# roclark/torchsr

Measured on AMD Instinct MI355X. Metric: 96x96 HR crops/sec (SRGAN GAN train step), higher is better.
Workload: dtype f32; 1 GPU; SRGAN full GAN step (Generator + Discriminator + VGG19 perceptual loss), 96x96 HR crops, batch 16 per GPU, fp32; per_gpu_batch=16, global_batch=16, crop=96, parallelism=dp1, hip_graph=True, vgg19_weights=seeded-random, plan_cus=256

## Files before the change

include/srx.h:

```cpp
#ifndef SRX_H
#define SRX_H

#include <stddef.h>
#include <stdint.h>

#ifdef __cplusplus
extern "C" {
#endif

#define SRX_VERSION 100

enum {
  SRX_OK = 0,
  SRX_E_BADARG = 1,
  SRX_E_UNSUPPORTED = 2,
  SRX_E_HIP = 3,
  SRX_E_WORKSPACE = 4
};

enum { SRX_ACT_NONE = 0, SRX_ACT_RELU = 1, SRX_ACT_LRELU = 2, SRX_ACT_PRELU = 3 };

int srx_version(void);
int srx_last_error(char* buf, size_t n);
int srx_build_info(char* buf, size_t n);
// ... 33 lines not shown
  int32_t up;
  int32_t precision;
} srx_conv2d_t;

size_t srx_conv2d_packed_fwd_floats(const srx_conv2d_t* d);
size_t srx_conv2d_packed_bwd_floats(const srx_conv2d_t* d);
size_t srx_conv2d_fwd_ws_floats(const srx_conv2d_t* d);
size_t srx_conv2d_bwd_data_ws_floats(const srx_conv2d_t* d);
size_t srx_conv2d_bwd_weight_ws_floats(const srx_conv2d_t* d);
int srx_conv2d_stat_rows(const srx_conv2d_t* d);

int srx_conv2d_plan(const srx_conv2d_t* d, int which, int* out);

int srx_conv2d_force_plan(int bm, int bn, int split, int ks);
int srx_conv2d_force_s2(int mode, int bm, int bn);
int srx_wgrad_force(int lin, int nsplit);
int srx_wgrad_force_kernels(int dma, int rows, int reduce);
int srx_thin_force_rows(int rows);
int srx_linear_force(int form, int splits);

int srx_thin_plan(const srx_conv2d_t* d, int which, int* out);

int srx_linear_plan(int B, int K, int J, int which, int* out);

int srx_wgrad_plan(const srx_conv2d_t* d, int nprob, int per_out, int* out);

int srx_conv2d_pack(const srx_conv2d_t* d, const float* w_oihw, float* wpk_fwd, float* wpk_bwd, void* stream);

size_t srx_pack_table_bytes(int n_layers);
int srx_pack_table_build(const srx_conv2d_t* descs, int n, const float* const* w_oihw, float* const* wpk_fwd,
// ... 279 lines not shown
```

torchsr_amd/_lib.py:

```python
import ctypes as C
import os
import subprocess
import sys

_HERE = os.path.dirname(os.path.abspath(__file__))
CSRC = os.path.join(_HERE, 'csrc')
LIB_PATH = os.environ.get('SRX_LIB') or os.path.join(CSRC, 'libsrx_hip.so')
SOURCES = ['api.cpp', 'gconv.hip', 'wgrad.hip', 'convpack.hip', 'c64.hip', 'thin9.hip', 'rdb.hip', 'thin.hip', 'rowtile.hip', 'augment.hip', 'degrade.hip', 'norm.hip', 'eltwise.hip', 'linear.hip', 'loss.hip', 'head.hip', 'wino.hip', 'optim.hip', 'dihedral.hip', 'resample.hip', 'usm.hip', 'pool.hip', 'colorfix.hip', 'compact.hip', 'specnorm.hip']
HEADERS = ['srx_common.h', 'conv_host.h', os.path.join('..', '..', 'include', 'srx.h')]

ACT_NONE, ACT_RELU, ACT_LRELU, ACT_PRELU = 0, 1, 2, 3


class Conv2dDesc(C.Structure):
    _fields_ = [
        ('N', C.c_int32), ('H', C.c_int32), ('W', C.c_int32),
        ('Cin', C.c_int32), ('Cin_s', C.c_int32), ('Cout', C.c_int32), ('Cout_s', C.c_int32),
        ('KH', C.c_int32), ('KW', C.c_int32), ('stride', C.c_int32), ('pad', C.c_int32),
        ('shuffle', C.c_int32), ('act', C.c_int32), ('slope', C.c_float), ('up', C.c_int32),
        ('precision', C.c_int32),
    ]


class DgradEpilogue(C.Structure):
# ... 118 lines not shown
    'srx_color_fix_wavelet_level': (_I, [_P, _P, _P, _P, _L, _I, _I, _I, _P]),
    'srx_plane_moments_blocks': (_I, [_I, _I]),
    'srx_plane_moments': (_I, [_P, _L, _I, _I, _P, _Z, _P, _P]),
    'srx_color_fix_adain_apply': (_I, [_P, _P, _L, _I, _I, _P, _P, _P]),
    'srx_conv2d_packed_fwd_floats': (_Z, [_D]),
    'srx_conv2d_packed_bwd_floats': (_Z, [_D]),
    'srx_conv2d_fwd_ws_floats': (_Z, [_D]),
    'srx_conv2d_bwd_data_ws_floats': (_Z, [_D]),
    'srx_conv2d_bwd_weight_ws_floats': (_Z, [_D]),
    'srx_conv2d_stat_rows': (_I, [_D]),
    'srx_conv2d_plan': (_I, [_D, _I, C.POINTER(C.c_int)]),
    'srx_conv2d_force_plan': (_I, [_I, _I, _I, _I]),
    'srx_thin_plan': (_I, [_D, _I, C.POINTER(C.c_int)]),
    'srx_thin_force_rows': (_I, [_I]),
    'srx_conv2d_force_s2': (_I, [_I, _I, _I]),
    'srx_wgrad_force': (_I, [_I, _I]),
    'srx_wgrad_force_kernels': (_I, [_I, _I, _I]),
    'srx_wgrad_plan': (_I, [_D, _I, _I, C.POINTER(C.c_int)]),
    'srx_linear_force': (_I, [_I, _I]),
    'srx_linear_plan': (_I, [_I, _I, _I, _I, C.POINTER(C.c_int)]),
    'srx_pack_table_bytes': (_Z, [_I]),
    'srx_pack_table_build': (_I, [_P, _I, _P, _P, _P, _P, C.POINTER(C.c_int), C.POINTER(C.c_longlong)]),
    'srx_pack_table_add_wino': (_I, [_P, C.POINTER(C.c_int), C.POINTER(C.c_longlong), _D, _P, _P, _I]),
    'srx_pack_table_run': (_I, [_P, _I, C.c_longlong, _P]),
    'srx_conv2d_pack': (_I, [_D, _P, _P, _P, _P]),
    'srx_conv2d_fwd': (_I, [_D, _P, _P, _P, _P, _P, _P, _Z, _P]),
    'srx_conv3x3_c64_bf16_packed_bytes': (_Z, [_I]),
    'srx_conv3x3_c64_bf16_pack': (_I, [_P, _P, _P, _I, _I, _P, _P]),
    'srx_conv3x3_c64_bf16_fwd': (_I, [_I, _I, _I, _I, _I, _P, _P, _F, _P, _P, _I, _P]),
    'srx_conv3x3_c64_bf16_plan': (_I, [_I, _I, _I, _I, C.POINTER(C.c_int)]),
# ... 202 lines not shown
```

torchsr_amd/csrc/api.cpp:

```cpp
#include "srx_common.h"
#include <cstdarg>
#include <cstdio>
#include <atomic>
#include <cstdlib>
#include <cstring>
#include <mutex>
#include <vector>

static thread_local char g_err[512] = "";

void srx_set_error(const char* fmt, ...) {
  va_list ap;
  va_start(ap, fmt);
  vsnprintf(g_err, sizeof(g_err), fmt, ap);
  va_end(ap);
}

extern "C" int srx_version(void) { return SRX_VERSION; }

#ifndef SRX_SOURCES_SHA256
#define SRX_SOURCES_SHA256 "unknown"
#endif
static const char g_build_info[] = "srx-build-sources-sha256:" SRX_SOURCES_SHA256;
extern "C" int srx_build_info(char* buf, size_t n) {
// ... 3 lines not shown
  return SRX_OK;
}

static SrxDevSwitches read_switches() {
  SrxDevSwitches s{};
  auto flag = [](const char* n) { const char* e = getenv(n); return e != nullptr && e[0] != 0 && !(e[0] == '0' && e[1] == 0); };
  auto num = [](const char* n) { const char* e = getenv(n); return e ? atoi(e) : 0; };
  s.no_rt36 = flag("SRX_NO_RT36");
  s.no_wgrad_rows = flag("SRX_NO_WGRAD_ROWS");
  s.no_bn_bwd_fuse = flag("SRX_NO_BN_BWD_FUSE");
  s.no_bn_fwd_fuse = flag("SRX_NO_BN_FWD_FUSE");
  s.no_first3 = flag("SRX_NO_FIRST3");
  s.no_c64 = flag("SRX_NO_C64");
  s.no_wgrad_dma = flag("SRX_NO_WGRAD_DMA");
  s.no_wgrad_lin = flag("SRX_NO_WGRAD_LIN");
  s.wgrad_nsplit = num("SRX_WGRAD_NSPLIT");
  s.wgrad_rows_nsplit = num("SRX_WGRAD_ROWS_NSPLIT");
  s.first3_wgs_per_cu = num("SRX_FIRST3_WGS_PER_CU");
  s.thin_fwd_rows = num("SRX_THIN_FWD_ROWS");
  s.reserved_cus = num("SRX_RESERVED_CUS");
  s.c64_ablate = num("SRX_C64_ABLATE");
  s.rdb_ablate = num("SRX_RDB_ABLATE");
  s.no_wino = flag("SRX_NO_WINO");
  s.old_wgrad_reduce = flag("SRX_OLD_WGRAD_REDUCE");
  s.wino_no_tail = flag("SRX_WINO_NO_TAIL");
  s.wino_zsplit = num("SRX_WINO_ZSPLIT");
  s.wino_bn = num("SRX_WINO_BN");
  s.s2_mode = num("SRX_S2_MODE");
  if (s.rdb_ablate != 0 || s.c64_ablate != 0) {
    const char* ok = getenv("SRX_ALLOW_GARBAGE_RESULTS");
// ... 142 lines not shown
```

torchsr_amd/csrc/conv_host.h:

```cpp
#pragma once
#include "srx_common.h"
#include <atomic>

constexpr int BK = 32;

struct Geo {
  int Ho, Wo, Ck, K, Kp, Cnp, cps;
};

struct BwdClass {
  int ph, pw, nth, ntw, dminh, dminw, Hm, Wm, K, Kp;
  size_t woff;
};

int check_desc(const srx_conv2d_t* d);
bool small_enough(const srx_conv2d_t* d);
int pad_rows(int c);
Geo fwd_geo(const srx_conv2d_t* d);
int bwd_ck(const srx_conv2d_t* d);
int bwd_classes(const srx_conv2d_t* d, BwdClass* cls, size_t& total_floats);
srx_conv2d_t upsampled_desc(const srx_conv2d_t* d);
size_t upsampled_floats(const srx_conv2d_t* d);

struct ConvForce {
  std::atomic<int> plan[4];
  std::atomic<int> s2[3];
  std::atomic<int> wg[2];
  std::atomic<int> wg_rows;
  std::atomic<int> wk[3];
};
ConvForce& conv_force();
```

torchsr_amd/csrc/gconv.hip:

```cpp
#include "conv_host.h"
#include <cstdio>
#include <cstdlib>
#include <algorithm>
#include <mutex>
#include <type_traits>
#include <utility>
#include <vector>

namespace {

struct GArgs {
  const float* in; const float* w; const float* bias; float* out; float* part;
  int N, Hi, Wi, Ci;
  int Hm, Wm, M, HmWm;
  float inv_HmWm, inv_Wm;
  int in_stride, nth, ntw, dh0, dw0, Ck, K, Kp;
  int Cn, Cs;
  int Ho, Wo, Co;
  int out_stride, oh_off, ow_off;
  int out_shuffle, in_shuffle;
  int up;
  int act; float slope;
  int linear_out;
  int mtiles;
// ... 3 lines not shown
  unsigned w_bytes;
  int big;
  unsigned in_margin;
  const float* add;
  float oscale;
  int add_ld, add_hi;
  float ascale;
  const float* mask;
  float mask_slope;
  int mask_lo, mask_hi;
  int out16, mask16;
};

constexpr int INVALID = -20000;

template <int BM, int BN, int WM, int WN, int KS, int XR, int PR, int UP = 0, int BIG = 0>
__device__ __forceinline__ void gconv_body(const GArgs& a, const int bid) {
  static_assert(XR == 0 || (XR == 16 && KS == 1), "extra rows: 16, without the in-workgroup K split");
  static_assert(PR == 0 || XR == 0, "the 16-row extension is fp32 only");
  constexpr bool H16 = PR == 1 || PR == 3;
  constexpr int BKL = H16 ? BK / 2 : BK;
  constexpr int NS = H16 ? 2 : 4;
  constexpr int BMT = BM + XR;
  constexpr int TM = WM / 32, TN = WN / 32;
  constexpr int WAVES_N = BN / WN;
  constexpr int WAVES_M = BM / WM;
  constexpr int GT = WAVES_M * WAVES_N * 64;
  constexpr int NT = GT * KS;
  static_assert(NT == 256 || NT == 512, "4 or 8 waves per workgroup");
  constexpr int RPP = GT / 8;
  constexpr int RA = (BMT + RPP - 1) / RPP, RB = BN / RPP;
  static_assert(RA >= 1 && RB >= 1, "tile too small for the thread count");
// ... 44 lines not shown
  size_t tbase = 0;
  if constexpr (BIG) {
    int n, mh, mw;
    split_row(min(m0, a.M - 1), n, mh, mw);
    const size_t c0 = centre(n, mh * a.in_stride, mw * a.in_stride);
    tbase = c0 > a.in_margin ? c0 - a.in_margin : 0;
    const unsigned tb_in_lo = (unsigned)srx_uniform((int)(unsigned)(tbase & 0xffffffffu));
    const unsigned tb_in_hi = (unsigned)srx_uniform((int)(unsigned)(tbase >> 32));
    tbase = ((size_t)tb_in_hi << 32) | tb_in_lo;
  }
  const size_t in_left = a.in_bytes - tbase;
  const __amdgpu_buffer_rsrc_t rin = BIG ? srx_rsrc(reinterpret_cast<const char*>(a.in) + tbase, in_left > 0xfffffff0ull ? 0xfffffff0u : (unsigned)in_left)
                                         : srx_rsrc(a.in, (unsigned)a.in_bytes);
  const __amdgpu_buffer_rsrc_t rw = srx_rsrc(a.w, a.w_bytes);

  for (int e = kc_beg * 8 + (int)threadIdx.x; e < kc_end * 8; e += NT) {
    const int k = 4 * e;
    int2 ent;
    if (k < a.K) {
      const int tap = k / a.Ck, c = k - tap * a.Ck;
      const int th = tap / a.ntw, tw = tap - th * a.ntw;
      const int dh = a.dh0 + th, dw = a.dw0 + tw;
      int koff;
      if (UP) {
        koff = c;
      } else if (a.in_shuffle) {
        const int ij = c / a.in_shuffle, cc = c - ij * a.in_shuffle;
        koff = ((2 * dh + (ij >> 1)) * (2 * a.Wi) + 2 * dw + (ij & 1)) * a.Ci + cc;
      } else {
        koff = (dh * a.Wi + dw) * a.Ci + c;
      }
      ent.x = (int)((unsigned)(dh & 0xffff) | ((unsigned)dw << 16));
      ent.y = koff * 4;
    } else {
      ent.x = (INVALID & 0xffff);
      ent.y = 0;
    }
    ktab[e - kc_beg * 8] = ent;
  }

  int rih[RA], riw[RA];
  unsigned rbase[RA];
#pragma unroll
  for (int p = 0; p < RA; ++p) {
    const int m = m0 + r0 + RPP * p;
    if (m < a.M && r0 + RPP * p < BMT) {
      int n, mh, mw;
      split_row(m, n, mh, mw);
      const int ih0 = mh * a.in_stride, iw0 = mw * a.in_stride;
      rih[p] = ih0;
      riw[p] = iw0;
      if constexpr (BIG) {
        rbase[p] = (unsigned)(centre(n, ih0, iw0) - tbase);
      } else {
        rbase[p] = 4u * (unsigned)(UP ? n * (a.Hi >> 1) * (a.Wi >> 1) * a.Ci
                                   : a.in_shuffle ? ((n * 2 * a.Hi + 2 * ih0) * (2 * a.Wi) + 2 * iw0) * a.Ci
                                                  : ((n * a.Hi + ih0) * a.Wi + iw0) * a.Ci);
      }
    } else {
      rih[p] = INVALID; riw[p] = 0; rbase[p] = 0;
    }
  }
  unsigned wvoff[RB];
#pragma unroll
  for (int p = 0; p < RB; ++p) wvoff[p] = 4u * ((unsigned)(n0 + r0 + RPP * p) * (unsigned)a.Kp + q * 4);
  __syncthreads();

  f32x16 acc[TM][TN];
#pragma unroll
  for (int i = 0; i < TM; ++i)
#pragma unroll
    for (int j = 0; j < TN; ++j)
#pragma unroll
      for (int r = 0; r < 16; ++r) acc[i][j][r] = 0.f;

  f32x4 ra0[RA], rb0[RB], ra1[RA], rb1[RB], ra2[RA], rb2[RB];
  auto gload = [&](int kc, f32x4 (&ra)[RA], f32x4 (&rb)[RB]) {
    const bool live = kc < kc_end;
    const int2 kt = ktab[(live ? kc - kc_beg : 0) * 8 + q];
    const int dh = (int)(short)(kt.x & 0xffff), dw = kt.x >> 16;
    if (UP) {
#pragma unroll
      for (int p = 0; p < RA; ++p) {
        const int ih = rih[p] + dh, iw = riw[p] + dw;
        const bool ok = live && ((unsigned)ih < (unsigned)a.Hi) && ((unsigned)iw < (unsigned)a.Wi);
        const unsigned pix = 4u * (unsigned)(((ih >> 1) * (a.Wi >> 1) + (iw >> 1)) * a.Ci);
        ra[p] = srx_bload(rin, ok ? rbase[p] + pix + (unsigned)kt.y : 0xffffffffu, 0);
      }
    } else {
#pragma unroll
      for (int p = 0; p < RA; ++p) {
        const int ih = rih[p] + dh, iw = riw[p] + dw;
        const bool ok = live && ((unsigned)ih < (unsigned)a.Hi) && ((unsigned)iw < (unsigned)a.Wi);
// ... 368 lines not shown
    }
    __syncthreads();
    if (lead && tid < BN) {
      float s = 0.f, s2 = 0.f;
#pragma unroll
      for (int w = 0; w < RED_ROWS; ++w) { s += red[(w * BN + tid) * 2]; s2 += red[(w * BN + tid) * 2 + 1]; }
      const int col = n0 + tid;
      if (col < a.Cn) {
        a.part[((size_t)mt * a.Cn + col) * 2 + 0] = s;
        a.part[((size_t)mt * a.Cn + col) * 2 + 1] = s2;
      }
    }
  }
}

template <int BM, int BN, int WM, int WN, int KS, int XR, int PR, int BIG = 0>
__global__ __launch_bounds__((BM / WM) * (BN / WN) * 64 * KS) void gconv_kernel(const GArgs a) {
  if (a.up) gconv_body<BM, BN, WM, WN, KS, XR, PR, 1, BIG>(a, blockIdx.x);
  else gconv_body<BM, BN, WM, WN, KS, XR, PR, 0, BIG>(a, blockIdx.x);
}

struct GMulti {
  int n;
  int first[5];
  GArgs g[4];
};
template <int BM, int BN, int WM, int WN, int XR, int PR = 0, int KS = 1>
__global__ __launch_bounds__((BM / WM) * (BN / WN) * 64 * KS) void gconv_multi_kernel(const GMulti m) {
  int ci = 0;
  while (ci + 1 < m.n && (int)blockIdx.x >= m.first[ci + 1]) ++ci;
  const GArgs a = m.g[ci];
  gconv_body<BM, BN, WM, WN, KS, XR, PR>(a, blockIdx.x - m.first[ci]);
}

struct S2Class {
  int nth, ntw, dh0, dw0;
  int chunks, pstart;
  int oh_off, ow_off;
  unsigned wbase, kpb;
};
struct GFused {
  GArgs g;
  int nclass, cpt, ptotal;
  S2Class c[4];
};

template <int BM, int BN, int WM, int WN, int XR, int PR>
// ... 479 lines not shown
srx_conv2d_t upsampled_desc(const srx_conv2d_t* d) {
  srx_conv2d_t h = *d;
  h.up = 0; h.H = 2 * d->H; h.W = 2 * d->W;
  return h;
}
size_t upsampled_floats(const srx_conv2d_t* d) { return (size_t)d->N * 2 * d->H * 2 * d->W * d->Cin_s; }

ConvForce& conv_force() {
  static ConvForce* f = [] {
    ConvForce* s = new ConvForce;
    const SrxDevSwitches& e = srx_dev();
    for (int i = 0; i < 4; ++i) s->plan[i].store(e.force_plan ? e.plan[i] : 0);
    s->s2[0].store((e.s2_mode & 1) ? 1 : 0); s->s2[1].store(0); s->s2[2].store(0);
    s->wg[0].store(e.no_wgrad_lin ? 0 : -1); s->wg[1].store(e.wgrad_nsplit > 0 && e.wgrad_nsplit <= 64 ? e.wgrad_nsplit : 0);
    s->wg_rows.store(e.wgrad_rows_nsplit > 0 && e.wgrad_rows_nsplit <= 64 ? e.wgrad_rows_nsplit : 0);
    s->wk[0].store(e.no_wgrad_dma ? 0 : -1); s->wk[1].store(e.no_wgrad_rows ? 0 : -1); s->wk[2].store(e.old_wgrad_reduce ? 0 : -1);
    return s;
  }();
  return *f;
}

namespace {

struct Plan { int BM, BN, mtiles, ntiles, tiles, full, tail, split, kc_per_split, ks; float cost; bool refused; };

enum Family { F_GCONV, F_BIG, F_MULTI, F_S2F, NFAM };
constexpr unsigned char K1 = 1, K2 = 2, K4 = 4, K12 = K1 | K2;
struct Tile {
  int BM, BN, WM, WN, XR;
  float eff;
  unsigned char ks[NFAM][4];
};
constexpr Tile kTiles[] = {
    {144, 128, 64, 32, 16, 0.91f, {{K1}, {}, {K1}, {K1}}},
    {144, 64, 32, 32, 16, 0.82f, {{K1}, {}, {K1}, {K1}}},
    {128, 128, 64, 32, 0, 0.95f, {{K1, K1, K1, K1}, {K1, K1, 0, K1}, {K1, K1}, {K1, K1}}},
    {128, 64, 32, 32, 0, 0.85f, {{K1, K1, K1, K1}, {K1, K1, 0, K1}, {K1, K1}, {K1, K1}}},
    {64, 64, 32, 32, 0, 0.60f, {{K12, K12, K12, K12}, {}, {K12, K12}, {K1, K1}}},
    {128, 32, 32, 32, 0, 0.50f, {{K1, K1, 0, K1}, {K1, K1, 0, K1}, {K1, K1}, {}}},
    {64, 32, 32, 32, 0, 0.50f, {{K2, K4, 0, K4}}},
    {256, 128, 64, 64, 0, 1.08f, {{0, K1, K1, K1}}},
};
constexpr int NTILES = sizeof(kTiles) / sizeof(kTiles[0]);

const Tile* find_tile(int bm, int bn) {
  const Tile* t = std::find_if(kTiles, kTiles + NTILES, [&](const Tile& x) { return x.BM == bm && x.BN == bn; });
  return t != kTiles + NTILES ? t : nullptr;
}
bool has_tile(Family f, int bm, int bn, int ks, int pr) {
  const Tile* t = find_tile(bm, bn);
  return t && (t->ks[f][pr] & (ks ? ks : K1 | K2 | K4)) != 0;
}
bool tile_sides_known(Family f, int bm, int bn) {
  bool rows = false, cols = false;
  for (const Tile& t : kTiles)
    if (t.ks[f][0] | t.ks[f][1] | t.ks[f][2] | t.ks[f][3]) { rows |= t.BM == bm; cols |= t.BN == bn; }
  return rows && cols;
}
int tile_ks(const Tile& t, Family f, int pr, bool two) {
  const int have = t.ks[f][pr];
  return have == K12 ? (two ? 2 : 1) : have ? have : 1;
}
bool columns_fit(int Cnp, int bn) { return Cnp == 32 ? bn == 32 : (bn != 32 && Cnp % bn == 0); }

float tile_us(int bm, int bn, int chunks, float eff, bool bf16) {
  return 2.0f * bm * bn * (float)chunks * BK / (4 * 64 * 2.1e3f) / eff / (bf16 ? 3.0f : 1.0f);
}
// ... 57 lines not shown
      return p;
    }
    p.BM = bm; p.BN = bn; p.mtiles = (int)srx_cdiv(M, bm); p.ntiles = Cnp / bn; p.tiles = p.mtiles * p.ntiles;
    if (sp > 1 && can_split) { p.full = 0; p.tail = p.tiles; p.kc_per_split = (int)srx_cdiv(kchunks, sp); p.split = (int)srx_cdiv(kchunks, p.kc_per_split); }
    else { p.full = p.tiles; p.tail = 0; p.split = 1; p.kc_per_split = kchunks; }
    p.ks = tile_ks(*find_tile(bm, bn), F_GCONV, pr, ks == 2);
    return p;
  }
  const Tile* t = find_tile(best.BM, best.BN);
  best.ks = t ? tile_ks(*t, fam, pr, best.full + best.tail * best.split <= P && best.kc_per_split >= 4) : 1;
  return best;
}

size_t plan_ws_floats(const Plan& p) { return p.split > 1 ? (size_t)p.tail * p.split * p.BM * p.BN : 0; }

template <int BM, int BN, int WM, int WN, int KS, int XR, int PR = 0, int BIG = 0>
int launch_gconv(const GArgs& a, const Plan& p, hipStream_t st) {
  const int ktab_chunks = p.full > 0 || p.split == 1 ? a.kchunks : p.kc_per_split;
  const size_t lds = gconv_lds_bytes(BM + XR, BN, KS, PR, ktab_chunks);
  if (lds > 160 * 1024) SRX_FAIL(SRX_E_UNSUPPORTED, "conv2d: K range needs %zu bytes of LDS", lds);
  static std::once_flag once;
  std::call_once(once, [] {
    (void)hipFuncSetAttribute(reinterpret_cast<const void*>(&gconv_kernel<BM, BN, WM, WN, KS, XR, PR, BIG>),
                              hipFuncAttributeMaxDynamicSharedMemorySize, 160 * 1024);
  });
  dim3 grid(p.full + p.tail * p.split);
  char nm[112];
  if (srx_prof_on())
    snprintf(nm, sizeof(nm), "gconv_kernel<%d, %d, %d, %d, %d, %d, %d%s> MxNxK=%dx%dx%d", BM, BN, WM, WN, KS, XR, PR, BIG ? ", big" : "",
             a.M, a.Cn, PR == 2 ? 2 * a.K : a.K);
  SRX_LAUNCH_PROF(nm, 2.0 * a.M * a.Cn * (PR == 2 ? 2 * a.K : a.K), (gconv_kernel<BM, BN, WM, WN, KS, XR, PR, BIG>), grid,
                  dim3((BM / WM) * (BN / WN) * 64 * KS), lds, st, a);
  SRX_CHECK_LAUNCH("gconv_kernel");
  if (p.split > 1) {
    hipLaunchKernelGGL((tail_fixup_kernel<BM + XR, BN>), dim3(p.tail * (BN / 16)), dim3(256), 0, st, a);
    SRX_CHECK_LAUNCH("tail_fixup_kernel");
  }
  return SRX_OK;
}

template <int BM, int BN, int WM, int WN, int XR, int PR = 0, int KS = 1>
int launch_gconv_multi(const GMulti& m, size_t lds, hipStream_t st) {
  static std::once_flag once;
  std::call_once(once, [] {
    (void)hipFuncSetAttribute(reinterpret_cast<const void*>(&gconv_multi_kernel<BM, BN, WM, WN, XR, PR, KS>),
                              hipFuncAttributeMaxDynamicSharedMemorySize, 160 * 1024);
  });
  char nm[64];
  double fl = 0.0;
  if (srx_prof_on()) {
    snprintf(nm, sizeof(nm), "gconv_multi_kernel<%d, %d, %d, %d, %d, %d, %d>", BM, BN, WM, WN, XR, PR, KS);
    for (int i = 0; i < m.n; ++i) fl += 2.0 * m.g[i].M * m.g[i].Cn * m.g[i].K;
  }
  SRX_LAUNCH_PROF(nm, fl, (gconv_multi_kernel<BM, BN, WM, WN, XR, PR, KS>), dim3(m.first[m.n]), dim3((BM / WM) * (BN / WN) * 64 * KS),
                  lds, st, m);
  SRX_CHECK_LAUNCH("gconv_multi_kernel");
  return SRX_OK;
}

template <int BM, int BN, int WM, int WN, int XR, int PR>
int launch_gconv_s2f(const GFused& f, dim3 grid, size_t lds, double fl, hipStream_t st) {
  static std::once_flag once;
  std::call_once(once, [] {
    (void)hipFuncSetAttribute(reinterpret_cast<const void*>(&gconv_s2f_kernel<BM, BN, WM, WN, XR, PR>),
                              hipFuncAttributeMaxDynamicSharedMemorySize, 160 * 1024);
  });
  char nm[64];
  if (srx_prof_on()) snprintf(nm, sizeof(nm), "gconv_s2f_kernel<%d, %d, %d, %d, %d, %d>", BM, BN, WM, WN, XR, PR);
  SRX_LAUNCH_PROF(nm, fl, (gconv_s2f_kernel<BM, BN, WM, WN, XR, PR>), grid, dim3((BM / WM) * (BN / WN) * 64), lds, st, f);
  SRX_CHECK_LAUNCH("gconv_s2f_kernel");
  return SRX_OK;
}

struct TileKey { int bm, bn, ks, pr; };

template <int F, int I, int PR, int KS, class... A>
bool launch_if(const TileKey& k, int& rc, const A&... args) {
  constexpr Tile t = kTiles[I];
  if constexpr ((t.ks[F][PR] & KS) != 0) {
    if (k.bm != t.BM || k.bn != t.BN || k.ks != KS || k.pr != PR) return false;
    if constexpr (F == F_MULTI) rc = launch_gconv_multi<t.BM - t.XR, t.BN, t.WM, t.WN, t.XR, PR, KS>(args...);
    else if constexpr (F == F_S2F) rc = launch_gconv_s2f<t.BM - t.XR, t.BN, t.WM, t.WN, t.XR, PR>(args...);
    else rc = launch_gconv<t.BM - t.XR, t.BN, t.WM, t.WN, KS, t.XR, PR, F == F_BIG>(args...);
    return true;
  }
  return false;
}
using Listable = std::make_integer_sequence<int, NTILES * 12>;
template <int F, int... J, class... A>
bool launch_tile(std::integer_sequence<int, J...>, const TileKey& k, int& rc, const A&... args) {
  return (launch_if<F, J / 12, J / 3 % 4, 1 << J % 3>(k, rc, args...) || ...);
}

// ... 30 lines not shown
        const float t = tile_us(bm, bn, kch, 1.0f, bf16);
        const float cost = ks == 2 ? 6.5f + 0.5f * t / 0.8f : 1.0f + t / tile.eff;
        const int tiles = (int)srx_cdiv(m.g[c].M, bm) * (int)srx_cdiv(m.g[c].Cn, bn);
        for (int t = 0; t < tiles; ++t) {
          std::pop_heap(heap.begin(), heap.end(), later);
          heap.back() += cost;
          if (heap.back() > makespan) makespan = heap.back();
          std::push_heap(heap.begin(), heap.end(), later);
        }
      }
    if (makespan < best) { best = makespan; BM = bm; BN = bn; KS = ks; }
  }
  return best;
}

int run_gconv_multi(GMulti& m, int BM, int BN, int KS, hipStream_t st, int precision = 0) {
  std::stable_sort(m.g, m.g + m.n, [](const GArgs& x, const GArgs& y) { return x.Kp > y.Kp; });
  int maxk = 0;
  m.first[0] = 0;
  for (int i = 0; i < m.n; ++i) {
    GArgs& a = m.g[i];
    a.kchunks = a.Kp / BK;
    a.mtiles = (int)srx_cdiv(a.M, BM);
    a.kc_per_split = a.kchunks;
    a.tail_split = 1;
    a.ws = nullptr;
    const int tiles = a.mtiles * (int)srx_cdiv(a.Cn, BN);
    a.full_tiles = tiles;
    m.first[i + 1] = m.first[i] + tiles;
    if (a.kchunks > maxk) maxk = a.kchunks;
  }
  const int pr = precision ? 1 : 0;
  const size_t lds = gconv_lds_bytes(BM, BN, KS, pr, maxk);
  if (lds > 160 * 1024) SRX_FAIL(SRX_E_UNSUPPORTED, "conv2d: K range needs %zu bytes of LDS", lds);
  int rc = SRX_OK;
  if (launch_tile<F_MULTI>(Listable{}, {BM, BN, KS, pr}, rc, m, lds, st)) return rc;
  SRX_FAIL(SRX_E_UNSUPPORTED, "conv2d_bwd_data: no%s gconv_multi_kernel for tile %d x %d", pr ? " bf16" : "", BM, BN);
}

bool s2f_eligible(const srx_conv2d_t* d, const BwdClass* cls, int nc) {
  if (nc < 2 || nc > 4 || d->shuffle || d->up || d->precision > 1) return false;
  if (bwd_ck(d) % BK != 0 || pad_rows(d->Cin) % 64 != 0) return false;
  for (int i = 0; i < nc; ++i)
    if (cls[i].K == 0 || cls[i].Hm != cls[0].Hm || cls[i].Wm != cls[0].Wm || cls[i].Hm <= 0 || cls[i].Wm <= 0) return false;
  return true;
}

float s2f_tile(const srx_conv2d_t* d, const BwdClass* cls, int nc, int& BM, int& BN) {
  const int P = srx_plan_cus();
  const bool bf16 = d->precision != 0;
  const int Cnp = pad_rows(d->Cin);
// ... 29 lines not shown
    S2Class& k = f.c[i];
    k.nth = cls[i].nth; k.ntw = cls[i].ntw; k.dh0 = cls[i].dminh; k.dw0 = cls[i].dminw;
    k.chunks = cls[i].K / BK; k.pstart = pos;
    k.oh_off = cls[i].ph; k.ow_off = cls[i].pw;
    k.wbase = (unsigned)(cls[i].woff * sizeof(float)); k.kpb = (unsigned)(cls[i].Kp * sizeof(float));
    pos += (int)srx_roundup(k.chunks, 3);
    fl += 2.0 * shared.M * shared.Cn * cls[i].K;
  }
  f.ptotal = pos;
  const int Cnp = pad_rows(d->Cin);
  const int pr = d->precision != 0 ? 1 : 0;
  const size_t lds = s2f_lds_bytes(BM, BN, pr, pos);
  if (lds > 160 * 1024) SRX_FAIL(SRX_E_UNSUPPORTED, "conv2d_bwd_data: K range needs %zu bytes of LDS", lds);
  const dim3 grid((unsigned)(f.g.mtiles * (Cnp / BN)));
  int rc = SRX_OK;
  if (launch_tile<F_S2F>(Listable{}, {BM, BN, 1, pr}, rc, f, grid, lds, fl, st)) return rc;
  SRX_FAIL(SRX_E_UNSUPPORTED, "conv2d_bwd_data: internal: no fused-class instantiation for tile %d x %d", BM, BN);
}

int strided_dgrad_plan(const srx_conv2d_t* d, const BwdClass* cls, int nc, const GMulti& m, int& BM, int& BN, int& KS, bool& fused) {
  ConvForce& f = conv_force();
  const int mode = f.s2[0].load(std::memory_order_relaxed);
  const bool bf16 = d->precision != 0;
  const int Cnp = pad_rows(d->Cin);
  const bool eligible = m.n == nc && s2f_eligible(d, cls, nc);
  fused = false;
  if (mode == 2) {
    if (!eligible)
      SRX_FAIL(SRX_E_UNSUPPORTED, "conv2d_bwd_data: forced gconv_s2f_kernel refused: the layer needs 2..4 non-empty stride-parity "
                                  "classes on one grid (extents multiples of the stride), Cout and Cin in whole chunks, no shuffle / upsample");
    int bm = f.s2[1].load(std::memory_order_relaxed), bn = f.s2[2].load(std::memory_order_relaxed);
// ... 23 lines not shown
int run_gconv(GArgs& a, const Plan& p, float* ws, size_t ws_floats, hipStream_t st, int precision = 0) {
  if (p.refused) return SRX_E_UNSUPPORTED;
  a.kchunks = a.Kp / BK;
  const size_t need = plan_ws_floats(p);
  if (need && (!ws || need > ws_floats))
    SRX_FAIL(SRX_E_WORKSPACE, "conv2d: split-K workspace %zu < %zu floats", ws_floats, need);
  if (p.split > 1 && !a.linear_out) SRX_FAIL(SRX_E_UNSUPPORTED, "conv2d: internal: split plan on a strided output");
  a.mtiles = p.mtiles;
  a.kc_per_split = p.kc_per_split;
  a.full_tiles = p.full;
  a.tail_split = p.split;
  a.ws = ws;
  int rc = SRX_OK;
  if (a.big) {
    if (p.split > 1) SRX_FAIL(SRX_E_UNSUPPORTED, "conv2d: internal: split plan on a call above 2^24 pixels");
    if (launch_tile<F_BIG>(Listable{}, {p.BM, p.BN, p.ks, precision == 3 ? 3 : precision ? 1 : 0}, rc, a, p, st)) return rc;
    SRX_FAIL(SRX_E_UNSUPPORTED, "conv2d: no whole-frame kernel for tile %dx%d", p.BM, p.BN);
  }
  if (launch_tile<F_GCONV>(Listable{}, {p.BM, p.BN, p.ks, precision}, rc, a, p, st)) return rc;
  static const char* const arith[4] = {"fp32", "bf16", "bf16-storage", "fp16"};
  SRX_FAIL(SRX_E_UNSUPPORTED, "conv2d: no %s kernel for tile %dx%d", arith[precision & 3], p.BM, p.BN);
}

void set_mgrid(GArgs& a, int N, int Hm, int Wm) {
  a.N = N; a.Hm = Hm; a.Wm = Wm; a.HmWm = Hm * Wm; a.M = N * Hm * Wm;
  a.inv_HmWm = 1.0f / (float)a.HmWm;
  a.inv_Wm = 1.0f / (float)Wm;
}

bool is_big(const srx_conv2d_t* d) { return !small_enough(d); }

Plan fwd_plan(const srx_conv2d_t* d, const Geo& g) {
  return make_plan(d->N * g.Ho * g.Wo, g.Cnp, g.Kp / BK, !d->shuffle, d->precision != 0, is_big(d));
}
// ... 98 lines not shown
              (tile_sides_known(F_GCONV, bm, bn) && split >= 1 && split <= 16 && (ks == 1 || ks == 2)),
              "conv2d_force_plan: (0, 0, 0, 0) or BM 64 / 128 / 144 / 256, BN 32 / 64 / 128, split 1..16, KS 1 / 2");
  ConvForce& f = conv_force();
  f.plan[1].store(0);
  f.plan[0].store(bm); f.plan[2].store(split); f.plan[3].store(ks); f.plan[1].store(bn);
  return SRX_OK;
}

extern "C" int srx_conv2d_force_s2(int mode, int bm, int bn) {
  SRX_REQUIRE(((mode == 0 || mode == 1) && bm == 0 && bn == 0) ||
              (mode == 2 && ((bm == 0 && bn == 0) || tile_sides_known(F_S2F, bm, bn))),
              "conv2d_force_s2: (0, 0, 0), (1, 0, 0) or (2, BM 64 / 128 / 144, BN 64 / 128) -- (2, 0, 0): the model's fused tile");
  ConvForce& f = conv_force();
  f.s2[0].store(0);
  f.s2[1].store(bm); f.s2[2].store(bn); f.s2[0].store(mode);
  return SRX_OK;
}

extern "C" int srx_wgrad_force(int lin, int nsplit) {
  SRX_REQUIRE(lin >= -1 && lin <= 1 && nsplit >= 0 && nsplit <= 64, "wgrad_force: LIN -1 / 0 / 1, 0..64 row splits");
  ConvForce& f = conv_force();
  f.wg[0].store(lin); f.wg[1].store(nsplit); f.wg_rows.store(nsplit);
  return SRX_OK;
}

extern "C" int srx_wgrad_force_kernels(int dma, int rows, int reduce) {
  SRX_REQUIRE(dma >= -1 && dma <= 1 && rows >= -1 && rows <= 1 && reduce >= -1 && reduce <= 1,
              "wgrad_force_kernels: DMA staging, image-row kernel, row-wise reduction: each -1 / 0 / 1");
  ConvForce& f = conv_force();
  f.wk[0].store(dma); f.wk[1].store(rows); f.wk[2].store(reduce);
// ... 367 lines not shown
```

torchsr_amd/csrc/srx_common.h:

```cpp
#pragma once
#include <hip/hip_runtime.h>
#include <hip/hip_ext.h>
#include <stdint.h>
#include <stddef.h>
#include "../../include/srx.h"

typedef float f32x4 __attribute__((ext_vector_type(4)));
typedef float f32x16 __attribute__((ext_vector_type(16)));

void srx_set_error(const char* fmt, ...);

#define SRX_FAIL(code, ...)      \
  do {                           \
    srx_set_error(__VA_ARGS__);  \
    return (code);               \
  } while (0)

#define SRX_REQUIRE(cond, ...) \
  do {                         \
    if (!(cond)) SRX_FAIL(SRX_E_BADARG, __VA_ARGS__); \
  } while (0)

#define SRX_CHECK_LAUNCH(name)                                                        \
  do {                                                                                \
    hipError_t e__ = hipGetLastError();                                               \
    if (e__ != hipSuccess) SRX_FAIL(SRX_E_HIP, "%s: %s", name, hipGetErrorString(e__)); \
  } while (0)

struct SrxDevSwitches {
  bool no_rt36, no_wgrad_rows, no_bn_bwd_fuse, no_bn_fwd_fuse, no_first3, no_c64, force_plan, no_wgrad_dma, no_wgrad_lin, no_wino, old_wgrad_reduce, wino_no_tail;
  int wgrad_nsplit, wgrad_rows_nsplit, first3_wgs_per_cu, thin_fwd_rows, reserved_cus, c64_ablate, rdb_ablate, wino_zsplit, wino_bn;
  int s2_mode;
  int plan[4];
};
const SrxDevSwitches& srx_dev();
extern "C" int srx_plan_cus(void);

bool srx_prof_on();
bool srx_prof_aux();
bool srx_prof_take(const char* name, double flops, hipEvent_t* e0, hipEvent_t* e1);
#define SRX_LAUNCH_PROF(name, flops, kernel, grid, block, lds, st, ...)                              \
  do {                                                                                               \
    hipEvent_t e0__ = nullptr, e1__ = nullptr;                                                       \
    if (srx_prof_on() && srx_prof_take(name, flops, &e0__, &e1__))                                   \
      hipExtLaunchKernelGGL(kernel, grid, block, (std::uint32_t)(lds), st, e0__, e1__, 0, __VA_ARGS__); \
// ... 91 lines not shown
```

Measured before the change: 2433 crops/s.

## Add tabled gather loader to gconv replacing LDS k-table with register tap walk

Adds a TAB variant of the implicit-GEMM conv body for plain fp32 non-upsampled convolutions. Instead of building a per-chunk (dh,dw) offset table in LDS and reading it on every load, each thread precomputes a per-row bitmask of in-image taps and walks tap/channel-chunk counters in scalar registers, using an out-of-range buffer offset to zero padding taps. The variant is enabled by default only for the 144-row tiles (single conv and multi-class dgrad) and can be disabled with an environment switch. It trades LDS traffic and address arithmetic for extra registers and is limited to at most 32 taps and Ck divisible by BK.

```diff
diff --git a/include/srx.h b/include/srx.h
--- a/include/srx.h
+++ b/include/srx.h
@@ -71,6 +71,8 @@
 
 int srx_conv2d_force_plan(int bm, int bn, int split, int ks);
 int srx_conv2d_force_s2(int mode, int bm, int bn);
+int srx_conv2d_force_gather(int tab);
+int srx_conv2d_gather_plan(const srx_conv2d_t* d, int which, int* out);
 int srx_wgrad_force(int lin, int nsplit);
 int srx_wgrad_force_kernels(int dma, int rows, int reduce);
 int srx_thin_force_rows(int rows);
diff --git a/torchsr_amd/_lib.py b/torchsr_amd/_lib.py
--- a/torchsr_amd/_lib.py
+++ b/torchsr_amd/_lib.py
@@ -156,6 +156,8 @@
     'srx_thin_plan': (_I, [_D, _I, C.POINTER(C.c_int)]),
     'srx_thin_force_rows': (_I, [_I]),
     'srx_conv2d_force_s2': (_I, [_I, _I, _I]),
+    'srx_conv2d_force_gather': (_I, [_I]),
+    'srx_conv2d_gather_plan': (_I, [_D, _I, C.POINTER(C.c_int)]),
     'srx_wgrad_force': (_I, [_I, _I]),
     'srx_wgrad_force_kernels': (_I, [_I, _I, _I]),
     'srx_wgrad_plan': (_I, [_D, _I, _I, C.POINTER(C.c_int)]),
diff --git a/torchsr_amd/csrc/api.cpp b/torchsr_amd/csrc/api.cpp
--- a/torchsr_amd/csrc/api.cpp
+++ b/torchsr_amd/csrc/api.cpp
@@ -41,6 +41,7 @@
   s.no_c64 = flag("SRX_NO_C64");
   s.no_wgrad_dma = flag("SRX_NO_WGRAD_DMA");
   s.no_wgrad_lin = flag("SRX_NO_WGRAD_LIN");
+  s.no_gather_tab = flag("SRX_NO_GATHER_TAB");
   s.wgrad_nsplit = num("SRX_WGRAD_NSPLIT");
   s.wgrad_rows_nsplit = num("SRX_WGRAD_ROWS_NSPLIT");
   s.first3_wgs_per_cu = num("SRX_FIRST3_WGS_PER_CU");
diff --git a/torchsr_amd/csrc/conv_host.h b/torchsr_amd/csrc/conv_host.h
--- a/torchsr_amd/csrc/conv_host.h
+++ b/torchsr_amd/csrc/conv_host.h
@@ -25,6 +25,7 @@
 struct ConvForce {
   std::atomic<int> plan[4];
   std::atomic<int> s2[3];
+  std::atomic<int> tab;
   std::atomic<int> wg[2];
   std::atomic<int> wg_rows;
   std::atomic<int> wk[3];
diff --git a/torchsr_amd/csrc/gconv.hip b/torchsr_amd/csrc/gconv.hip
--- a/torchsr_amd/csrc/gconv.hip
+++ b/torchsr_amd/csrc/gconv.hip
@@ -41,8 +41,9 @@
 
 constexpr int INVALID = -20000;
 
-template <int BM, int BN, int WM, int WN, int KS, int XR, int PR, int UP = 0, int BIG = 0>
+template <int BM, int BN, int WM, int WN, int KS, int XR, int PR, int UP = 0, int BIG = 0, int TAB = 0>
 __device__ __forceinline__ void gconv_body(const GArgs& a, const int bid) {
+  static_assert(TAB == 0 || (PR == 0 && UP == 0 && BIG == 0), "the tabled loader: plain fp32 gathers below 2^24 pixels");
   static_assert(XR == 0 || (XR == 16 && KS == 1), "extra rows: 16, without the in-workgroup K split");
   static_assert(PR == 0 || XR == 0, "the 16-row extension is fp32 only");
   constexpr bool H16 = PR == 1 || PR == 3;
@@ -117,7 +118,7 @@
                                          : srx_rsrc(a.in, (unsigned)a.in_bytes);
   const __amdgpu_buffer_rsrc_t rw = srx_rsrc(a.w, a.w_bytes);
 
-  for (int e = kc_beg * 8 + (int)threadIdx.x; e < kc_end * 8; e += NT) {
+  for (int e = kc_beg * 8 + (int)threadIdx.x; !TAB && e < kc_end * 8; e += NT) {
     const int k = 4 * e;
     int2 ent;
     if (k < a.K) {
@@ -144,6 +145,12 @@
 
   int rih[RA], riw[RA];
   unsigned rbase[RA];
+  int rout_of[RA];
+  unsigned rows1 = 0;
+  if constexpr (TAB) {
+    for (int th = 0; th < a.nth; ++th) rows1 |= 1u << (th * a.ntw);
+  }
+  auto below = [](int n) -> unsigned { return (unsigned)((1ull << n) - 1ull); };
 #pragma unroll
   for (int p = 0; p < RA; ++p) {
     const int m = m0 + r0 + RPP * p;
@@ -153,7 +160,15 @@
       const int ih0 = mh * a.in_stride, iw0 = mw * a.in_stride;
       rih[p] = ih0;
       riw[p] = iw0;
-      if constexpr (BIG) {
+      if constexpr (TAB) {
+        const int eh = ih0 + a.dh0, ew = iw0 + a.dw0;
+        const int hl = min(max(-eh, 0), a.nth), hh = max(min(a.Hi - eh, a.nth), hl);
+        const int wl = min(max(-ew, 0), a.ntw), wh = max(min(a.Wi - ew, a.ntw), wl);
+        const unsigned wbits = below(wh) & ~below(wl);
+        const unsigned in_img = (wbits * rows1) & below(hh * a.ntw) & ~below(hl * a.ntw);
+        rout_of[p] = (int)~in_img;
+        rbase[p] = 4u * (unsigned)(((n * a.Hi + ih0) * a.Wi + iw0) * a.Ci) + 16u * (unsigned)q;
+      } else if constexpr (BIG) {
         rbase[p] = (unsigned)(centre(n, ih0, iw0) - tbase);
       } else {
         rbase[p] = 4u * (unsigned)(UP ? n * (a.Hi >> 1) * (a.Wi >> 1) * a.Ci
@@ -162,7 +177,19 @@
       }
     } else {
       rih[p] = INVALID; riw[p] = 0; rbase[p] = 0;
-    }
+      if constexpr (TAB) rout_of[p] = -1;
+    }
+  }
+  const int cpt = TAB ? a.Ck / BK : 1;
+  int tb_t = 0, tb_th = 0, tb_tw = 0, tb_c = 0;
+  int tb_ones = -1;
+  if constexpr (TAB) asm("" : "+s"(tb_ones));
+  if constexpr (TAB) {
+    const int first = kc_beg + ks;
+    tb_t = srx_uniform(first / cpt);
+    tb_c = first - tb_t * cpt;
+    tb_th = srx_uniform(tb_t / a.ntw);
+    tb_tw = tb_t - tb_th * a.ntw;
   }
   unsigned wvoff[RB];
 #pragma unroll
@@ -180,6 +207,23 @@
   f32x4 ra0[RA], rb0[RB], ra1[RA], rb1[RB], ra2[RA], rb2[RB];
   auto gload = [&](int kc, f32x4 (&ra)[RA], f32x4 (&rb)[RB]) {
     const bool live = kc < kc_end;
+    if constexpr (TAB) {
+      const unsigned koff = 4u * (unsigned)(((a.dh0 + tb_th) * a.Wi + a.dw0 + tb_tw) * a.Ci + tb_c * BK);
+      const int dead = live ? 0 : tb_ones;
+#pragma unroll
+      for (int p = 0; p < RA; ++p)
+        ra[p] = srx_bload(rin, (rbase[p] + koff) | (unsigned)(__builtin_amdgcn_sbfe(rout_of[p], (unsigned)tb_t, 1u) | dead), 0);
+#pragma unroll
+      for (int p = 0; p < RB; ++p)
+        rb[p] = srx_bload(rw, live ? wvoff[p] : 0xffffffffu, (unsigned)srx_uniform(live ? kc * (BK * 4) : 0));
+#pragma unroll
+      for (int i = 0; i < KS; ++i)
+        if (++tb_c == cpt) {
+          tb_c = 0; ++tb_t;
+          if (++tb_tw == a.ntw) { tb_tw = 0; ++tb_th; }
+        }
+      return;
+    }
     const int2 kt = ktab[(live ? kc - kc_beg : 0) * 8 + q];
     const int dh = (int)(short)(kt.x & 0xffff), dw = kt.x >> 16;
     if (UP) {
@@ -578,8 +622,9 @@
   }
 }
 
-template <int BM, int BN, int WM, int WN, int KS, int XR, int PR, int BIG = 0>
+template <int BM, int BN, int WM, int WN, int KS, int XR, int PR, int BIG = 0, int TAB = 0>
 __global__ __launch_bounds__((BM / WM) * (BN / WN) * 64 * KS) void gconv_kernel(const GArgs a) {
+  if constexpr (TAB) { gconv_body<BM, BN, WM, WN, KS, XR, PR, 0, BIG, 1>(a, blockIdx.x); return; }
   if (a.up) gconv_body<BM, BN, WM, WN, KS, XR, PR, 1, BIG>(a, blockIdx.x);
   else gconv_body<BM, BN, WM, WN, KS, XR, PR, 0, BIG>(a, blockIdx.x);
 }
@@ -589,12 +634,12 @@
   int first[5];
   GArgs g[4];
 };
-template <int BM, int BN, int WM, int WN, int XR, int PR = 0, int KS = 1>
+template <int BM, int BN, int WM, int WN, int XR, int PR = 0, int KS = 1, int TAB = 0>
 __global__ __launch_bounds__((BM / WM) * (BN / WN) * 64 * KS) void gconv_multi_kernel(const GMulti m) {
   int ci = 0;
   while (ci + 1 < m.n && (int)blockIdx.x >= m.first[ci + 1]) ++ci;
   const GArgs a = m.g[ci];
-  gconv_body<BM, BN, WM, WN, KS, XR, PR>(a, blockIdx.x - m.first[ci]);
+  gconv_body<BM, BN, WM, WN, KS, XR, PR, 0, 0, TAB>(a, blockIdx.x - m.first[ci]);
 }
 
 struct S2Class {
@@ -1104,6 +1149,7 @@
     s->s2[0].store((e.s2_mode & 1) ? 1 : 0); s->s2[1].store(0); s->s2[2].store(0);
     s->wg[0].store(e.no_wgrad_lin ? 0 : -1); s->wg[1].store(e.wgrad_nsplit > 0 && e.wgrad_nsplit <= 64 ? e.wgrad_nsplit : 0);
     s->wg_rows.store(e.wgrad_rows_nsplit > 0 && e.wgrad_rows_nsplit <= 64 ? e.wgrad_rows_nsplit : 0);
+    s->tab.store(e.no_gather_tab ? 0 : -1);
     s->wk[0].store(e.no_wgrad_dma ? 0 : -1); s->wk[1].store(e.no_wgrad_rows ? 0 : -1); s->wk[2].store(e.old_wgrad_reduce ? 0 : -1);
     return s;
   }();
@@ -1120,16 +1166,17 @@
   int BM, BN, WM, WN, XR;
   float eff;
   unsigned char ks[NFAM][4];
+  unsigned char tab[2];
 };
 constexpr Tile kTiles[] = {
-    {144, 128, 64, 32, 16, 0.91f, {{K1}, {}, {K1}, {K1}}},
-    {144, 64, 32, 32, 16, 0.82f, {{K1}, {}, {K1}, {K1}}},
-    {128, 128, 64, 32, 0, 0.95f, {{K1, K1, K1, K1}, {K1, K1, 0, K1}, {K1, K1}, {K1, K1}}},
-    {128, 64, 32, 32, 0, 0.85f, {{K1, K1, K1, K1}, {K1, K1, 0, K1}, {K1, K1}, {K1, K1}}},
-    {64, 64, 32, 32, 0, 0.60f, {{K12, K12, K12, K12}, {}, {K12, K12}, {K1, K1}}},
-    {128, 32, 32, 32, 0, 0.50f, {{K1, K1, 0, K1}, {K1, K1, 0, K1}, {K1, K1}, {}}},
-    {64, 32, 32, 32, 0, 0.50f, {{K2, K4, 0, K4}}},
-    {256, 128, 64, 64, 0, 1.08f, {{0, K1, K1, K1}}},
+    {144, 128, 64, 32, 16, 0.91f, {{K1}, {}, {K1}, {K1}}, {K1, K1}},
+    {144, 64, 32, 32, 16, 0.82f, {{K1}, {}, {K1}, {K1}}, {K1, K1}},
+    {128, 128, 64, 32, 0, 0.95f, {{K1, K1, K1, K1}, {K1, K1, 0, K1}, {K1, K1}, {K1, K1}}, {}},
+    {128, 64, 32, 32, 0, 0.85f, {{K1, K1, K1, K1}, {K1, K1, 0, K1}, {K1, K1}, {K1, K1}}, {}},
+    {64, 64, 32, 32, 0, 0.60f, {{K12, K12, K12, K12}, {}, {K12, K12}, {K1, K1}}, {}},
+    {128, 32, 32, 32, 0, 0.50f, {{K1, K1, 0, K1}, {K1, K1, 0, K1}, {K1, K1}, {}}, {}},
+    {64, 32, 32, 32, 0, 0.50f, {{K2, K4, 0, K4}}, {}},
+    {256, 128, 64, 64, 0, 1.08f, {{0, K1, K1, K1}}, {}},
 };
 constexpr int NTILES = sizeof(kTiles) / sizeof(kTiles[0]);
 
@@ -1141,6 +1188,18 @@
   const Tile* t = find_tile(bm, bn);
   return t && (t->ks[f][pr] & (ks ? ks : K1 | K2 | K4)) != 0;
 }
+bool has_tab_tile(Family f, int bm, int bn, int ks) {
+  const Tile* t = find_tile(bm, bn);
+  return t && (f == F_GCONV || f == F_MULTI) && (t->tab[f == F_MULTI] & ks) != 0;
+}
+bool gather_tab_eligible(int precision, int in_shuffle, int up, int big, int Ck, int taps) {
+  return precision == 0 && !in_shuffle && !up && !big && Ck % BK == 0 && taps >= 1 && taps <= 32;
+}
+bool gather_tab_eligible(const GArgs& a, int precision) {
+  return gather_tab_eligible(precision, a.in_shuffle, a.up, a.big, a.Ck, a.nth * a.ntw) && a.K == a.Kp;
+}
+bool gather_tab_wanted() { return conv_force().tab.load(std::memory_order_relaxed) != 0; }
+
 bool tile_sides_known(Family f, int bm, int bn) {
   bool rows = false, cols = false;
   for (const Tile& t : kTiles)
@@ -1228,14 +1287,14 @@
 
 size_t plan_ws_floats(const Plan& p) { return p.split > 1 ? (size_t)p.tail * p.split * p.BM * p.BN : 0; }
 
-template <int BM, int BN, int WM, int WN, int KS, int XR, int PR = 0, int BIG = 0>
+template <int BM, int BN, int WM, int WN, int KS, int XR, int PR = 0, int BIG = 0, int TAB = 0>
 int launch_gconv(const GArgs& a, const Plan& p, hipStream_t st) {
   const int ktab_chunks = p.full > 0 || p.split == 1 ? a.kchunks : p.kc_per_split;
   const size_t lds = gconv_lds_bytes(BM + XR, BN, KS, PR, ktab_chunks);
   if (lds > 160 * 1024) SRX_FAIL(SRX_E_UNSUPPORTED, "conv2d: K range needs %zu bytes of LDS", lds);
   static std::once_flag once;
   std::call_once(once, [] {
-    (void)hipFuncSetAttribute(reinterpret_cast<const void*>(&gconv_kernel<BM, BN, WM, WN, KS, XR, PR, BIG>),
+    (void)hipFuncSetAttribute(reinterpret_cast<const void*>(&gconv_kernel<BM, BN, WM, WN, KS, XR, PR, BIG, TAB>),
                               hipFuncAttributeMaxDynamicSharedMemorySize, 160 * 1024);
   });
   dim3 grid(p.full + p.tail * p.split);
@@ -1243,7 +1302,7 @@
   if (srx_prof_on())
     snprintf(nm, sizeof(nm), "gconv_kernel<%d, %d, %d, %d, %d, %d, %d%s> MxNxK=%dx%dx%d", BM, BN, WM, WN, KS, XR, PR, BIG ? ", big" : "",
              a.M, a.Cn, PR == 2 ? 2 * a.K : a.K);
-  SRX_LAUNCH_PROF(nm, 2.0 * a.M * a.Cn * (PR == 2 ? 2 * a.K : a.K), (gconv_kernel<BM, BN, WM, WN, KS, XR, PR, BIG>), grid,
+  SRX_LAUNCH_PROF(nm, 2.0 * a.M * a.Cn * (PR == 2 ? 2 * a.K : a.K), (gconv_kernel<BM, BN, WM, WN, KS, XR, PR, BIG, TAB>), grid,
                   dim3((BM / WM) * (BN / WN) * 64 * KS), lds, st, a);
   SRX_CHECK_LAUNCH("gconv_kernel");
   if (p.split > 1) {
@@ -1253,11 +1312,11 @@
   return SRX_OK;
 }
 
-template <int BM, int BN, int WM, int WN, int XR, int PR = 0, int KS = 1>
+template <int BM, int BN, int WM, int WN, int XR, int PR = 0, int KS = 1, int TAB = 0>
 int launch_gconv_multi(const GMulti& m, size_t lds, hipStream_t st) {
   static std::once_flag once;
   std::call_once(once, [] {
-    (void)hipFuncSetAttribute(reinterpret_cast<const void*>(&gconv_multi_kernel<BM, BN, WM, WN, XR, PR, KS>),
+    (void)hipFuncSetAttribute(reinterpret_cast<const void*>(&gconv_multi_kernel<BM, BN, WM, WN, XR, PR, KS, TAB>),
                               hipFuncAttributeMaxDynamicSharedMemorySize, 160 * 1024);
   });
   char nm[64];
@@ -1266,7 +1325,7 @@
     snprintf(nm, sizeof(nm), "gconv_multi_kernel<%d, %d, %d, %d, %d, %d, %d>", BM, BN, WM, WN, XR, PR, KS);
     for (int i = 0; i < m.n; ++i) fl += 2.0 * m.g[i].M * m.g[i].Cn * m.g[i].K;
   }
-  SRX_LAUNCH_PROF(nm, fl, (gconv_multi_kernel<BM, BN, WM, WN, XR, PR, KS>), dim3(m.first[m.n]), dim3((BM / WM) * (BN / WN) * 64 * KS),
+  SRX_LAUNCH_PROF(nm, fl, (gconv_multi_kernel<BM, BN, WM, WN, XR, PR, KS, TAB>), dim3(m.first[m.n]), dim3((BM / WM) * (BN / WN) * 64 * KS),
                   lds, st, m);
   SRX_CHECK_LAUNCH("gconv_multi_kernel");
   return SRX_OK;
@@ -1286,11 +1345,19 @@
   return SRX_OK;
 }
 
-struct TileKey { int bm, bn, ks, pr; };
+struct TileKey { int bm, bn, ks, pr, tab; };
 
 template <int F, int I, int PR, int KS, class... A>
 bool launch_if(const TileKey& k, int& rc, const A&... args) {
   constexpr Tile t = kTiles[I];
+  if constexpr ((F == F_GCONV || F == F_MULTI) && PR == 0 && (t.tab[F == F_MULTI] & KS) != 0) {
+    static_assert((t.ks[F][0] & KS) != 0, "a tabled kernel without its plain form");
+    if (k.tab && k.bm == t.BM && k.bn == t.BN && k.ks == KS && k.pr == 0) {
+      if constexpr (F == F_MULTI) rc = launch_gconv_multi<t.BM - t.XR, t.BN, t.WM, t.WN, t.XR, 0, KS, 1>(args...);
+      else rc = launch_gconv<t.BM - t.XR, t.BN, t.WM, t.WN, KS, t.XR, 0, 0, 1>(args...);
+      return true;
+    }
+  }
   if constexpr ((t.ks[F][PR] & KS) != 0) {
     if (k.bm != t.BM || k.bn != t.BN || k.ks != KS || k.pr != PR) return false;
     if constexpr (F == F_MULTI) rc = launch_gconv_multi<t.BM - t.XR, t.BN, t.WM, t.WN, t.XR, PR, KS>(args...);
@@ -1351,6 +1418,13 @@
   return best;
 }
 
+int multi_tabled(const GMulti& m, int BM, int BN, int KS, int precision) {
+  if (!gather_tab_wanted() || !has_tab_tile(F_MULTI, BM, BN, KS)) return 0;
+  for (int i = 0; i < m.n; ++i)
+    if (!gather_tab_eligible(m.g[i], precision)) return 0;
+  return 1;
+}
+
 int run_gconv_multi(GMulti& m, int BM, int BN, int KS, hipStream_t st, int precision = 0) {
   std::stable_sort(m.g, m.g + m.n, [](const GArgs& x, const GArgs& y) { return x.Kp > y.Kp; });
   int maxk = 0;
@@ -1371,7 +1445,7 @@
   const size_t lds = gconv_lds_bytes(BM, BN, KS, pr, maxk);
   if (lds > 160 * 1024) SRX_FAIL(SRX_E_UNSUPPORTED, "conv2d: K range needs %zu bytes of LDS", lds);
   int rc = SRX_OK;
-  if (launch_tile<F_MULTI>(Listable{}, {BM, BN, KS, pr}, rc, m, lds, st)) return rc;
+  if (launch_tile<F_MULTI>(Listable{}, {BM, BN, KS, pr, multi_tabled(m, BM, BN, KS, precision)}, rc, m, lds, st)) return rc;
   SRX_FAIL(SRX_E_UNSUPPORTED, "conv2d_bwd_data: no%s gconv_multi_kernel for tile %d x %d", pr ? " bf16" : "", BM, BN);
 }
 
@@ -1431,7 +1505,7 @@
   if (lds > 160 * 1024) SRX_FAIL(SRX_E_UNSUPPORTED, "conv2d_bwd_data: K range needs %zu bytes of LDS", lds);
   const dim3 grid((unsigned)(f.g.mtiles * (Cnp / BN)));
   int rc = SRX_OK;
-  if (launch_tile<F_S2F>(Listable{}, {BM, BN, 1, pr}, rc, f, grid, lds, fl, st)) return rc;
+  if (launch_tile<F_S2F>(Listable{}, {BM, BN, 1, pr, 0}, rc, f, grid, lds, fl, st)) return rc;
   SRX_FAIL(SRX_E_UNSUPPORTED, "conv2d_bwd_data: internal: no fused-class instantiation for tile %d x %d", BM, BN);
 }
 
@@ -1485,10 +1559,11 @@
   int rc = SRX_OK;
   if (a.big) {
     if (p.split > 1) SRX_FAIL(SRX_E_UNSUPPORTED, "conv2d: internal: split plan on a call above 2^24 pixels");
-    if (launch_tile<F_BIG>(Listable{}, {p.BM, p.BN, p.ks, precision == 3 ? 3 : precision ? 1 : 0}, rc, a, p, st)) return rc;
+    if (launch_tile<F_BIG>(Listable{}, {p.BM, p.BN, p.ks, precision == 3 ? 3 : precision ? 1 : 0, 0}, rc, a, p, st)) return rc;
     SRX_FAIL(SRX_E_UNSUPPORTED, "conv2d: no whole-frame kernel for tile %dx%d", p.BM, p.BN);
   }
-  if (launch_tile<F_GCONV>(Listable{}, {p.BM, p.BN, p.ks, precision}, rc, a, p, st)) return rc;
+  const int tab = gather_tab_wanted() && gather_tab_eligible(a, precision) && has_tab_tile(F_GCONV, p.BM, p.BN, p.ks);
+  if (launch_tile<F_GCONV>(Listable{}, {p.BM, p.BN, p.ks, precision, tab}, rc, a, p, st)) return rc;
   static const char* const arith[4] = {"fp32", "bf16", "bf16-storage", "fp16"};
   SRX_FAIL(SRX_E_UNSUPPORTED, "conv2d: no %s kernel for tile %dx%d", arith[precision & 3], p.BM, p.BN);
 }
@@ -1617,6 +1692,36 @@
   ConvForce& f = conv_force();
   f.s2[0].store(0);
   f.s2[1].store(bm); f.s2[2].store(bn); f.s2[0].store(mode);
+  return SRX_OK;
+}
+
+extern "C" int srx_conv2d_force_gather(int tab) {
+  SRX_REQUIRE(tab >= -1 && tab <= 1, "conv2d_force_gather: -1 / 1 (the tabled loader where eligible) or 0 (never)");
+  conv_force().tab.store(tab);
+  return SRX_OK;
+}
+
+extern "C" int srx_conv2d_gather_plan(const srx_conv2d_t* d, int which, int* out) {
+  if (int rc = check_desc(d)) return rc;
+  SRX_REQUIRE(out && (which == 0 || which == 1), "conv2d_gather_plan: null pointer / which must be 0 or 1");
+  const srx_conv2d_t h = which == 1 && d->up == 2 ? upsampled_desc(d) : *d;
+  int pl[6];
+  if (int rc = srx_conv2d_plan(&h, which, pl)) return rc;
+  out[0] = 0;
+  if (!gather_tab_wanted() || srx_rt36_applicable(&h)) return SRX_OK;
+  if (which == 0) {
+    if (srx_thin_fwd_applicable(&h) || srx_first3_fwd_applicable(&h)) return SRX_OK;
+    const Geo g = fwd_geo(&h);
+    out[0] = gather_tab_eligible(h.precision, 0, h.up == 2, is_big(&h), g.Ck, h.KH * h.KW) && has_tab_tile(F_GCONV, pl[0], pl[1], pl[4]);
+    return SRX_OK;
+  }
+  if (srx_thin_dgrad_applicable(&h) || pl[5] == 2) return SRX_OK;
+  BwdClass cls[16];
+  size_t total;
+  const int nc = bwd_classes(&h, cls, total);
+  int taps = 1;
+  for (int i = 0; i < nc; ++i) taps = std::max(taps, cls[i].nth * cls[i].ntw);
+  out[0] = gather_tab_eligible(h.precision, h.shuffle, 0, 0, bwd_ck(&h), taps) && has_tab_tile(pl[5] == 1 ? F_MULTI : F_GCONV, pl[0], pl[1], pl[4]);
   return SRX_OK;
 }
 
diff --git a/torchsr_amd/csrc/srx_common.h b/torchsr_amd/csrc/srx_common.h
--- a/torchsr_amd/csrc/srx_common.h
+++ b/torchsr_amd/csrc/srx_common.h
@@ -28,7 +28,7 @@
   } while (0)
 
 struct SrxDevSwitches {
-  bool no_rt36, no_wgrad_rows, no_bn_bwd_fuse, no_bn_fwd_fuse, no_first3, no_c64, force_plan, no_wgrad_dma, no_wgrad_lin, no_wino, old_wgrad_reduce, wino_no_tail;
+  bool no_rt36, no_wgrad_rows, no_bn_bwd_fuse, no_bn_fwd_fuse, no_first3, no_c64, force_plan, no_wgrad_dma, no_wgrad_lin, no_wino, old_wgrad_reduce, wino_no_tail, no_gather_tab;
   int wgrad_nsplit, wgrad_rows_nsplit, first3_wgs_per_cu, thin_fwd_rows, reserved_cus, c64_ablate, rdb_ablate, wino_zsplit, wino_bn;
   int s2_mode;
   int plan[4];
```

Result: no change. 2429 crops/s (-0.2%).
